# yl4579/StyleTTS2

Hardware: AMD Instinct MI355X
Metric: audio-seconds/sec (RTF^-1) end-to-end, 10 s utterance batch (higher is better)
Workload: dtype f32 (convs/linears: f16 hi/lo split, 3 MFMA products, fp32 accumulate)

## Files before the change

### include/st2.h

```cpp
#ifndef ST2_H
#define ST2_H

#include <stdint.h>

#ifdef __cplusplus
extern "C" {
#endif

#define ST2_ABI_VERSION 23

int st2_abi_version(void);
const char* st2_last_error(void);
int st2_device_info(int dev, char* name, int cap);

#define ST2_STATUS_F16_RANGE 1
#define ST2_STATUS_LSTM_TIMEOUT 2
#define ST2_STATUS_DURATION_SUM 4
#define ST2_STATUS_LSTM_RECOVERED 8
#define ST2_STATUS_FRAME_CAPACITY 16
int st2_status(int clear);

enum st2_prologue {
  ST2_PRO_NONE = 0,
  ST2_PRO_LEAKY = 1,
// ... 275 lines not shown
int st2_durations_fit(const int64_t* dur, int32_t B, int32_t N, const int32_t* len, const int32_t* target, const uint8_t* hold,
                      int32_t T_cap, int64_t* out, int32_t* report, void* stream);

int64_t st2_clip_ingest_work_bytes(int32_t B, int32_t L_cap);
int st2_clip_ingest(const void* src, int64_t src_bs, const int32_t* n, int32_t B, int32_t N_cap, int32_t fmt, int32_t up,
                    int32_t down, const float* taps, int32_t taps_per_phase, float top_db, int32_t L_min, float* wave,
                    int64_t w_bs, int32_t L_cap, int32_t* len, int32_t* start, int32_t* flags, void* work, int64_t work_bytes,
                    void* stream);

int st2_stft_frames(const float* wave, int64_t w_bs, int32_t B, int32_t L, int32_t n_win, int32_t hop, int32_t shift,
                    float* frames, int64_t f_bs, int32_t f_cs, void* stream);
int st2_power_spectrum(const float* y, int64_t y_bs, int32_t y_cs, int32_t B, int32_t K, int32_t M, float* p,
                       int64_t p_bs, int32_t p_cs, void* stream);
int st2_log_norm(float* x, int64_t n, float eps, float mean, float stdv, void* stream);
int st2_dwconv3x3s2(const float* x, int64_t x_bs, int64_t x_hs, int32_t x_cs, const float* w, const float* bias,
                    int32_t B, int32_t C, int32_t H, int32_t W, float* y, int64_t y_bs, int64_t y_hs, int32_t y_cs,
                    void* stream);
int st2_avgpool2x2(const float* x, int64_t x_bs, int64_t x_hs, int32_t x_cs, int32_t B, int32_t C, int32_t H, int32_t W,
                   float* y, int64_t y_bs, int64_t y_hs, int32_t y_cs, void* stream);

int st2_axpbypcz(const float* x, float a, const float* y, float b, const float* z, float c,
                 float* out, int64_t n, void* stream);

typedef struct st2_engine st2_engine;

typedef struct st2_model_config {
  int32_t decoder_kind;
  int32_t dim_in;
  int32_t style_dim;
  int32_t upsample_initial_channel;
  int32_t n_upsamples;  int32_t upsample_rates[4];  int32_t upsample_kernel_sizes[4];
  int32_t n_resblock_kernels;  int32_t resblock_kernel_sizes[4];  int32_t resblock_dilations[4][3];
  int32_t gen_istft_n_fft, gen_istft_hop;
  int32_t multispeaker;
  int32_t dn_layers, dn_heads, dn_head_features, dn_multiplier;
  int32_t dn_channels;
  int32_t dn_embedding;
  int32_t dn_context_features;
  int32_t dn_max_length;
  int32_t pred_hidden;
  int32_t bert_layers;
  float bert_ln_eps;
} st2_model_config;

int st2_create(const st2_model_config* cfg, st2_engine** out);
int st2_destroy(st2_engine* e);
// ... 184 lines not shown
```

### styletts2_amd/_lib.py

```python
import ctypes as C
import os

import torch

_HERE = os.path.dirname(os.path.abspath(__file__))
LIB_PATH = os.path.join(_HERE, "libst2_hip.so")
ABI_VERSION = 23
HEADROOM_COLS, CALIBRATION_COLS = 12, 5

f32p = C.c_void_p

PRO_NONE, PRO_LEAKY, PRO_ADAIN_LEAKY, PRO_ADAIN_SNAKE, PRO_SNAKE, PRO_COLNORM = range(6)
STATUS_F16_RANGE, STATUS_LSTM_TIMEOUT, STATUS_DURATION_SUM, STATUS_LSTM_RECOVERED = 1, 2, 4, 8
STATUS_FRAME_CAPACITY = 16
PACK_F32, PACK_S16 = 0, 1
PCM_F32, PCM_S16, PCM_ULAW, PCM_ALAW = range(4)
NOISE_NORMAL, NOISE_BITS = 0, 1
NOISE_SAMPLER, NOISE_STEP, NOISE_SINE = 0, 1, 0x10000
ACT_NONE, ACT_GELU, ACT_EXP_SIN, ACT_TANH, ACT_LEAKY, ACT_GELU_TANH = range(6)


class ConvDesc(C.Structure):
    _fields_ = [
        ("B", C.c_int32), ("C_in", C.c_int32), ("C_out", C.c_int32), ("L_in", C.c_int32),
# ... 294 lines not shown
    "st2_probe_mfma_stream": (C.c_int, [C.c_int32, C.c_int32, C.c_int32, C.c_void_p]),
    "st2_debug_headroom": (C.c_int, [C.c_int]),
    "st2_debug_headroom_read": (C.c_int, [C.POINTER(C.c_double), C.c_int32]),
    "st2_conv1d_xs_part_cols": (C.c_int, [C.POINTER(ConvDesc)]),
    "st2_conv1d_f16s_set_splitk": (None, [C.c_int, C.c_int]),
    "st2_calibrate": (C.c_int, [C.c_void_p, C.c_int32, C.POINTER(C.c_int32)]),
    "st2_calibration_read": (C.c_int, [C.c_void_p, C.POINTER(C.c_double), C.c_int32]),
    "st2_calibration_site_name": (C.c_int, [C.c_void_p, C.c_int32, C.c_char_p, C.c_int32]),
    "st2_calibration_write": (C.c_int, [C.c_void_p, C.POINTER(C.c_float), C.c_int32]),
    "st2_calibration_scale": (C.c_float, [C.c_float, C.c_int32]),
    "st2_stream_create_cu_mask": (C.c_int, [C.POINTER(C.c_uint32), C.c_int32, C.POINTER(C.c_void_p)]),
    "st2_stream_destroy": (C.c_int, [C.c_void_p]),
    "st2_debug_set_backend": (C.c_int, [C.POINTER(C.c_void_p), C.c_int32]),
    "st2_stft_frames": (C.c_int, [f32p, C.c_int64, C.c_int32, C.c_int32, C.c_int32, C.c_int32, C.c_int32, f32p,
                                  C.c_int64, C.c_int32, C.c_void_p]),
    "st2_power_spectrum": (C.c_int, [f32p, C.c_int64, C.c_int32, C.c_int32, C.c_int32, C.c_int32, f32p, C.c_int64,
                                     C.c_int32, C.c_void_p]),
    "st2_log_norm": (C.c_int, [f32p, C.c_int64, C.c_float, C.c_float, C.c_float, C.c_void_p]),
    "st2_dwconv3x3s2": (C.c_int, [f32p, C.c_int64, C.c_int64, C.c_int32, f32p, f32p, C.c_int32, C.c_int32, C.c_int32,
                                  C.c_int32, f32p, C.c_int64, C.c_int64, C.c_int32, C.c_void_p]),
    "st2_avgpool2x2": (C.c_int, [f32p, C.c_int64, C.c_int64, C.c_int32, C.c_int32, C.c_int32, C.c_int32, C.c_int32, f32p,
                                 C.c_int64, C.c_int64, C.c_int32, C.c_void_p]),
    "st2_axpbypcz": (C.c_int, [f32p, C.c_float, f32p, C.c_float, f32p, C.c_float, f32p, C.c_int64, C.c_void_p]),
    "st2_stft_frames_len": (C.c_int, [f32p, C.c_int64, C.c_int32, C.c_int32, C.c_int32, C.c_int32, C.c_int32, f32p,
                                      C.c_int64, C.c_int32, C.c_void_p, C.c_int32, C.c_void_p, C.c_void_p]),
    "st2_log_norm_len": (C.c_int, [f32p, C.c_int64, C.c_int32, C.c_int32, C.c_int32, C.c_int32, C.c_float, C.c_float,
                                   C.c_float, C.c_void_p, C.c_void_p]),
    "st2_dwconv3x3s2_len": (C.c_int, [f32p, C.c_int64, C.c_int64, C.c_int32, f32p, f32p, C.c_int32, C.c_int32, C.c_int32,
                                      C.c_int32, f32p, C.c_int64, C.c_int64, C.c_int32, C.c_void_p, C.c_void_p]),
    "st2_avgpool2x2_len": (C.c_int, [f32p, C.c_int64, C.c_int64, C.c_int32, C.c_int32, C.c_int32, C.c_int32, C.c_int32, f32p,
                                     C.c_int64, C.c_int64, C.c_int32, C.c_void_p, C.c_void_p]),
    "st2_style_lengths_count": (C.c_int64, [C.c_int32, C.c_int32, C.c_int32]),
    "st2_style_lengths": (C.c_int, [C.c_void_p, C.c_int32, C.c_int32, C.c_int32, C.c_int32, C.c_int32, C.c_void_p,
                                    C.c_void_p]),
    "st2_style_workspace_bytes_ragged": (C.c_int64, [C.c_void_p, C.c_int32, C.c_int32, C.c_int32, C.c_int32]),
    "st2_style_forward_ragged": (C.c_int, [C.c_void_p, C.c_int32, f32p, C.c_void_p, C.c_int32, C.c_int32, C.c_int32, f32p,
                                           C.c_void_p, C.c_int64, C.c_void_p]),
    "st2_conv_launch_plan": (C.c_int, [C.POINTER(ConvDesc), C.c_int32, C.c_int32, C.c_int32, C.POINTER(ConvPlan)]),
    "st2_convt_interleave_part_cols": (C.c_int, []),
}

EXPORTS = tuple(_SIGNATURES)
_lib = None


class St2Error(RuntimeError):
# ... 44 lines not shown
```

### styletts2_amd/csrc/st2_glue.hip

```cpp
#include <string.h>

#include "st2_common.h"

namespace {

__global__ __launch_bounds__(256) void time_features_kernel(float t, const float* __restrict__ w, int H2, int B,
                                                            float* __restrict__ out) {
  const int j = blockIdx.x * 256 + threadIdx.x;
  const int b = blockIdx.y;
  const int W = 1 + 2 * H2;
  if (j >= W) return;
  float v;
  if (j == 0) {
    v = t;
  } else {
    const int k = (j - 1) % H2;
    const float f = ((t * w[k]) * 2.0f) * 3.14159274101257324f;
    v = (j - 1) < H2 ? sinf(f) : cosf(f);
  }
  out[(int64_t)b * W + j] = v;
}

__global__ __launch_bounds__(256) void tokens_to_channels_kernel(const float* __restrict__ e, int64_t e_bs, int N, int E,
                                                                 float* __restrict__ y, int64_t y_bs, int y_cs) {
// ... 155 lines not shown
  const int tx = threadIdx.x & 31, ty = threadIdx.x >> 5;
  const int nlen = len ? len[b] : N;
#pragma unroll
  for (int i = 0; i < 4; ++i) {
    const int n = n0 + ty + 8 * i, e = e0 + tx;
    float v = 0.f;
    if (n < N && n < nlen && e < E) {
      const long long t = tok[(int64_t)b * N + n];
      if (t >= 0 && t < V) v = table[t * E + e];
      if (add) v += add[e];
      if (pos) v += pos[(int64_t)n * E + e];
    }
    tile[ty + 8 * i][tx] = v;
  }
  __syncthreads();
  float* yb = y + (int64_t)b * y_bs;
#pragma unroll
  for (int i = 0; i < 4; ++i) {
    const int e = e0 + ty + 8 * i, n = n0 + tx;
    if (n < N && e < E) yb[(int64_t)e * y_cs + n] = tile[tx][ty + 8 * i];
  }
}

}

extern "C" int st2_embed_tokens(const int64_t* tokens, int32_t B, int32_t N, const float* table, int32_t V, int32_t E,
                                const float* add, const float* pos, const int32_t* len, float* y, int64_t y_bs,
                                int32_t y_cs, void* stream) {
  ST2_REQUIRE(tokens && table && y && B > 0 && N > 0 && V > 0 && E > 0, "st2_embed_tokens: bad arguments");
  ST2_REQUIRE(B <= 65535, "st2_embed_tokens: grid too large");
  hipLaunchKernelGGL(embed_tokens_kernel, dim3(st2_cdiv(N, 32), st2_cdiv(E, 32), B), dim3(256), 0,
                     reinterpret_cast<hipStream_t>(stream), reinterpret_cast<const long long*>(tokens), table, V, E, N, add,
                     pos, len, y, y_bs, y_cs);
  ST2_CHECK_LAUNCH("st2_embed_tokens");
  return 0;
}

extern "C" int st2_mask_tail(float* x, int64_t x_bs, int32_t x_cs, int32_t B, int32_t C, int32_t L, const int32_t* len,
                             void* stream) {
  ST2_REQUIRE(x && len && B > 0 && C > 0 && L > 0, "st2_mask_tail: bad arguments");
  ST2_REQUIRE(B <= 65535 && C <= 65535, "st2_mask_tail: grid too large");
  hipLaunchKernelGGL(mask_tail_kernel, dim3(st2_cdiv(L, 256), C, B), dim3(256), 0, reinterpret_cast<hipStream_t>(stream), x,
                     x_bs, x_cs, L, len);
  ST2_CHECK_LAUNCH("st2_mask_tail");
  return 0;
}
// ... 113 lines not shown
```

### styletts2_amd/csrc/st2_norm.hip

```cpp
#include "st2_common.h"

namespace {

template <int NT>
__global__ __launch_bounds__(NT) void instnorm_stats_kernel(const float* __restrict__ x, int64_t x_bs, int x_cs,
                                                            int C, int L_max, float eps, float* __restrict__ stats,
                                                            const int32_t* __restrict__ len) {
  const int row = blockIdx.x;
  const int b = row / C;
  const int c = row % C;
  const int L = len ? min(max(len[b], 1), L_max) : L_max;
  const float* xr = x + (int64_t)b * x_bs + (int64_t)c * x_cs;
  double s = 0.0, ss = 0.0;
  if ((reinterpret_cast<uintptr_t>(xr) & 15) == 0) {
    typedef float f4 __attribute__((ext_vector_type(4)));
    double a[4] = {0.0, 0.0, 0.0, 0.0}, q[4] = {0.0, 0.0, 0.0, 0.0};
    const int L4 = L >> 2;
    const f4* x4 = reinterpret_cast<const f4*>(xr);
    for (int i = threadIdx.x; i < L4; i += NT) {
      const f4 v = x4[i];
#pragma unroll
      for (int e = 0; e < 4; ++e) {
        const double d = (double)v[e];
        a[e] += d;
// ... 37 lines not shown
  __shared__ double red[2][NT / 64];
  const int lane = threadIdx.x & 63, wave = threadIdx.x >> 6;
  if (lane == 0) {
    red[0][wave] = s;
    red[1][wave] = ss;
  }
  __syncthreads();
  if (threadIdx.x == 0) {
    double ts = 0.0, tss = 0.0;
#pragma unroll
    for (int w = 0; w < NT / 64; ++w) {
      ts += red[0][w];
      tss += red[1][w];
    }
    const double mean = ts / (double)L;
    double var = tss / (double)L - mean * mean;
    if (var < 0.0) var = 0.0;
    stats[(int64_t)row * 2 + 0] = (float)mean;
    stats[(int64_t)row * 2 + 1] = (float)(1.0 / sqrt(var + (double)eps));
  }
}

constexpr int CW = 16;
__global__ __launch_bounds__(64 * CW) void colnorm_stats_kernel(const float* __restrict__ x, int64_t x_bs, int x_cs,
                                                                int C, int L, float eps, float* __restrict__ stats) {
  __shared__ double red[2][CW][64];
  const int lane = threadIdx.x & 63;
  const int w = threadIdx.x >> 6;
  const int l = blockIdx.x * 64 + lane;
  const int b = blockIdx.y;
  const bool live = l < L;
  const float* xb = x + (int64_t)b * x_bs + (live ? l : 0);
  double s = 0.0, ss = 0.0;
  int c = w;
  for (; c + 7 * CW < C; c += 8 * CW) {
    float v[8];
#pragma unroll
    for (int u = 0; u < 8; ++u) v[u] = xb[(int64_t)(c + u * CW) * x_cs];
#pragma unroll
    for (int u = 0; u < 8; ++u) {
      const double dv = (double)v[u];
      s += dv;
      ss += dv * dv;
    }
  }
  for (; c < C; c += CW) {
    const double dv = (double)xb[(int64_t)c * x_cs];
    s += dv;
    ss += dv * dv;
  }
  red[0][w][lane] = s;
  red[1][w][lane] = ss;
  __syncthreads();
  if (w == 0 && live) {
    double ts = 0.0, tss = 0.0;
#pragma unroll
    for (int i = 0; i < CW; ++i) {
      ts += red[0][i][lane];
      tss += red[1][i][lane];
    }
    const double mean = ts / (double)C;
    double var = tss / (double)C - mean * mean;
    if (var < 0.0) var = 0.0;
    float* o = stats + ((int64_t)b * L + l) * 2;
    o[0] = (float)mean;
    o[1] = (float)(1.0 / sqrt(var + (double)eps));
  }
}

constexpr int FC_BT = 8;
constexpr int FC_J = 64;
constexpr int FC_KS = 16;
constexpr int FC_NT = FC_J * FC_KS;
__global__ __launch_bounds__(FC_NT) void style_fc_kernel(const float* __restrict__ s, int B, int K,
                                                       const float* __restrict__ wt, const float* __restrict__ bias,
                                                       int J, int act, float* __restrict__ h) {
  extern __shared__ __attribute__((aligned(16))) float sl[];
  float* red = sl + FC_BT * K;
  const int jj = threadIdx.x & (FC_J - 1);
  const int ks = threadIdx.x / FC_J;
  const int j = blockIdx.x * FC_J + jj;
  const int jc = min(j, J - 1);
  const int b0 = blockIdx.y * FC_BT;
  const int nb = min(FC_BT, B - b0);
  for (int e = threadIdx.x; e < FC_BT * K; e += FC_NT) {
    const int bb = e / K, k = e % K;
    sl[e] = bb < nb ? s[(int64_t)(b0 + bb) * K + k] : 0.f;
  }
  __syncthreads();
  float acc[FC_BT];
// ... 96 lines not shown
extern "C" int st2_instnorm_stats_len(const float* x, int64_t x_bs, int32_t x_cs, int32_t B, int32_t C, int32_t L,
                                      float eps, float* stats, const int32_t* len, void* stream) {
  ST2_REQUIRE(x && stats && B > 0 && C > 0 && L > 0, "st2_instnorm_stats: bad arguments");
  hipStream_t s = reinterpret_cast<hipStream_t>(stream);
  const int rows = B * C;
  if (L <= 2048)
    hipLaunchKernelGGL((instnorm_stats_kernel<64>), dim3(rows), dim3(64), 0, s, x, x_bs, x_cs, C, L, eps, stats, len);
  else
    hipLaunchKernelGGL((instnorm_stats_kernel<256>), dim3(rows), dim3(256), 0, s, x, x_bs, x_cs, C, L, eps, stats, len);
  ST2_CHECK_LAUNCH("st2_instnorm_stats");
  return 0;
}

extern "C" int st2_colnorm_stats(const float* x, int64_t x_bs, int32_t x_cs, int32_t B, int32_t C, int32_t L,
                                 float eps, float* stats, void* stream) {
  ST2_REQUIRE(x && stats && B > 0 && C > 0 && L > 0, "st2_colnorm_stats: bad arguments");
  hipStream_t s = reinterpret_cast<hipStream_t>(stream);
  hipLaunchKernelGGL(colnorm_stats_kernel, dim3(st2_cdiv(L, 64), B), dim3(64 * CW), 0, s, x, x_bs, x_cs, C, L, eps,
                     stats);
  ST2_CHECK_LAUNCH("st2_colnorm_stats");
  return 0;
}

extern "C" int st2_style_fc(const float* sv, int32_t B, int32_t K, const float* wt, const float* bias, int32_t J,
                            int32_t act, float* h, void* stream) {
  ST2_REQUIRE(sv && wt && h && B > 0 && K > 0 && J > 0, "st2_style_fc: bad arguments");
  ST2_REQUIRE(K <= 2048, "st2_style_fc: K=%d too large", K);
  ST2_REQUIRE(act == ST2_ACT_NONE || act == ST2_ACT_GELU, "st2_style_fc: act must be NONE or GELU");
  hipStream_t s = reinterpret_cast<hipStream_t>(stream);
  const size_t smem = ((size_t)FC_BT * K + (size_t)FC_KS * FC_BT * FC_J) * sizeof(float);
  static std::atomic<uint64_t> attr_done{0};
  st2_once_per_device(attr_done, [&] {
    (void)hipFuncSetAttribute(reinterpret_cast<const void*>(&style_fc_kernel), hipFuncAttributeMaxDynamicSharedMemorySize,
                              160 * 1024);
  });
  hipLaunchKernelGGL(style_fc_kernel, dim3(st2_cdiv(J, FC_J), st2_cdiv(B, FC_BT)), dim3(FC_NT), smem, s, sv, B, K, wt,
                     bias, J, act, h);
  ST2_CHECK_LAUNCH("st2_style_fc");
  return 0;
}
```

### styletts2_amd/csrc/st2_plan_sampler.inc

```

struct Sess {
  Ctx& c;
  const st2_engine& e;
  int B, N;
  bool merged;
  const int32_t* key_len;
  View bases[2];
  int nbases;
  const float* feat_map;
  const float* ada;
  double scale;
};

View dn_alloc(Sess& s, int C) {
  View v;
  v.B = s.B; v.C = C; v.L = s.N;
  v.p = s.c.a.f32((int64_t)s.B * C * s.N);
  if (s.merged) { v.bs = s.N; v.cs = s.B * s.N; } else { v.bs = (int64_t)C * s.N; v.cs = s.N; }
  return v;
}
View dn_cv(const Sess& s, const View& t) {
  if (!s.merged) return t;
  View v = t;
  v.B = 1; v.L = s.B * s.N; v.bs = (int64_t)t.C * v.L; v.cs = v.L;
  return v;
}

const float* dn_mapping(Sess& s, float c_noise) {
  Ctx& c = s.c;
  const st2_engine& e = s.e;
  const PDenoiser& d = e.dn;
  const int F = d.features, H2 = e.cfg.dn_channels / 2;
  float* four = c.a.f32((int64_t)s.B * (1 + 2 * H2));
  RUN(c, g_be.time_features(c_noise, e.F(d.time_w), H2, s.B, four, c.stream));
  float* m = c.a.f32((int64_t)s.B * F);
  RUN(c, g_be.style_fc(four, s.B, 1 + 2 * H2, e.F(d.time_lin), e.F(d.time_b), F, ST2_ACT_GELU, m, c.stream));
  if (s.feat_map) {
    float* m2 = c.a.f32((int64_t)s.B * F);
    RUN(c, g_be.axpbypcz(m, 1.0f, s.feat_map, 1.0f, nullptr, 0.0f, m2, (int64_t)s.B * F, c.stream));
    m = m2;
  }
  float* m3 = c.a.f32((int64_t)s.B * F);
  RUN(c, g_be.style_fc(m, s.B, F, e.F(d.map0), e.F(d.map0_b), F, ST2_ACT_GELU, m3, c.stream));
  float* m4 = c.a.f32((int64_t)s.B * F);
  RUN(c, g_be.style_fc(m3, s.B, F, e.F(d.map2), e.F(d.map2_b), F, ST2_ACT_GELU, m4, c.stream));
  return m4;
}

void dn_run(Sess& s, View base, const float* x, const float* m, float* out) {
  Ctx& c = s.c;
  const st2_engine& e = s.e;
  const PDenoiser& d = e.dn;
  const st2_model_config& cfg = e.cfg;
  const int B = s.B, N = s.N, Fz = d.features, C = cfg.dn_channels;
  const int mid = cfg.dn_heads * cfg.dn_head_features;
  const int64_t mark = c.a.off;
  View b0 = base.rows(0, C);
  RUN(c, g_be.broadcast_cols(x, C, b0.p, b0.bs, b0.cs, B, C, N, c.stream));
  View X = dn_alloc(s, Fz);
  RUN(c, g_be.add_chanvec(base.p, base.bs, base.cs, m, Fz, X.p, X.bs, X.cs, B, Fz, N, c.stream));
  const int nblk = (int)d.blocks.size();
  for (int i = 0; i < nblk; ++i) {
    const PBlock& b = d.blocks[(size_t)i];
    float* st = c.a.f32((int64_t)B * N * 2);
    RUN(c, g_be.colnorm_stats(X.p, X.bs, X.cs, B, Fz, N, 1e-5f, st, c.stream));
    View qkv = dn_alloc(s, 3 * mid);
    ConvOpt o1, o2;
    o1.pro = o2.pro = ST2_PRO_COLNORM;
    o1.stats = o2.stats = st;
    if (cfg.multispeaker) {
      const int64_t J = (int64_t)nblk * 4 * Fz;
      const float* a = s.ada + (int64_t)4 * Fz * i;
      o1.gamma = a;          o1.beta = a + Fz;     o1.gb_bs = J; o1.gamma_plus_one = 1;
      o2.gamma = a + 2 * Fz; o2.beta = a + 3 * Fz; o2.gb_bs = J; o2.gamma_plus_one = 1;
    } else {
      o1.gamma = e.F(b.n_w);  o1.beta = e.F(b.n_b);
      o2.gamma = e.F(b.nc_w); o2.beta = e.F(b.nc_b);
    }
    const bool seg = cfg.multispeaker && s.merged && B > 1 &&
                     conv_rule(ST2_PRO_COLNORM, 1, 1, Fz, mid, B * N).route == ST2_CONV_ROUTE_XS;
    if (seg) o1.gb_seg = o2.gb_seg = N;
    const bool per_utt = cfg.multispeaker && !seg;
    View Xv = per_utt ? X : dn_cv(s, X), qv = per_utt ? qkv : dn_cv(s, qkv);
    conv(c, e, Xv, b.q, qv.rows(0, mid), o1);
    conv(c, e, Xv, b.kv, qv.rows(mid, 3 * mid), o2);
    View att = dn_alloc(s, mid);
    View q = qkv.rows(0, mid), k = qkv.rows(mid, 2 * mid), v = qkv.rows(2 * mid, 3 * mid);
    RUN(c, g_be.attention_keylen(q.p, k.p, v.p, q.bs, q.cs, att.p, att.bs, att.cs, B, cfg.dn_heads, cfg.dn_head_features,
                                 N, (float)pow((double)cfg.dn_head_features, -0.5), s.key_len, c.stream));
    View X1 = dn_alloc(s, Fz), hmid = dn_alloc(s, b.f1_out), X2 = dn_alloc(s, Fz);
    ConvOpt oo;
    oo.bias = e.F(b.o_b); oo.res = dn_cv(s, X);
    conv(c, e, dn_cv(s, att), b.o, dn_cv(s, X1), oo);
    ConvOpt of1;
    of1.bias = e.F(b.f1_b); of1.act = ST2_ACT_GELU;
    conv(c, e, dn_cv(s, X1), b.f1, dn_cv(s, hmid), of1);
    ConvOpt of2;
    of2.bias = e.F(b.f2_b); of2.res = dn_cv(s, X1);
    conv(c, e, dn_cv(s, hmid), b.f2, dn_cv(s, X2), of2);
    if (i + 1 < nblk) {
      View Xn = dn_alloc(s, Fz);
      RUN(c, g_be.add_chanvec(X2.p, X2.bs, X2.cs, m, Fz, Xn.p, Xn.bs, Xn.cs, B, Fz, N, c.stream));
      X = Xn;
    } else {
      X = X2;
    }
  }
  float* mean = c.a.f32((int64_t)B * Fz);
  RUN(c, g_be.mean_tokens_len(X.p, X.bs, X.cs, mean, Fz, B, Fz, N, s.key_len, c.stream));
  RUN(c, g_be.style_fc(mean, B, Fz, e.F(d.out_t), e.F(d.out_b), C, ST2_ACT_NONE, out, c.stream));
  c.a.off = mark;
}

void dn_denoise(Sess& s, const float* x, const double* w4, float* out) {
  Ctx& c = s.c;
  const int C = s.e.cfg.dn_channels;
  const int64_t n = (int64_t)s.B * C;
  const int64_t mark = c.a.off;
  const float c_skip = (float)w4[0], c_out = (float)w4[1], c_in = (float)w4[2], c_noise = (float)w4[3];
  float* x_in = c.a.f32(n);
  RUN(c, g_be.axpbypcz(x, c_in, nullptr, 0.f, nullptr, 0.f, x_in, n, c.stream));
  const float* m = dn_mapping(s, c_noise);
  float* pred = c.a.f32(n);
  dn_run(s, s.bases[0], x_in, m, pred);
  if (s.nbases > 1) {
    float* pm = c.a.f32(n);
    dn_run(s, s.bases[1], x_in, m, pm);
    float* mix = c.a.f32(n);
    RUN(c, g_be.axpbypcz(pm, (float)(1.0 - s.scale), pred, (float)s.scale, nullptr, 0.f, mix, n, c.stream));
    pred = mix;
  }
  RUN(c, g_be.axpbypcz(x, c_skip, pred, c_out, nullptr, 0.f, out, n, c.stream));
  c.a.off = mark;
}

int sampler_plan(Ctx& c, const st2_engine& e, const float* noise, const float* embedding, const View* emb_cm,
                 const float* features, const float* step_noise, const int32_t* lengths, int B, int N, int steps, double scale,
                 const double* table, double sigma0, float* out, float* step_taps) {
  const st2_model_config& cfg = e.cfg;
  const PDenoiser& d = e.dn;
  const int C = cfg.dn_channels, E = cfg.dn_embedding, Fz = d.features;
  Sess s{c, e, B, N, true, lengths, {}, 1, nullptr, nullptr, scale};
  s.bases[0] = dn_alloc(s, Fz);
  {
    View dst = s.bases[0].rows(C, Fz);
    if (emb_cm)
      RUN(c, g_be.copy_ncl(emb_cm->p, emb_cm->bs, emb_cm->cs, dst.p, dst.bs, dst.cs, B, E, N, c.stream));
    else
      RUN(c, g_be.tokens_to_channels(embedding, (int64_t)N * E, B, N, E, dst.p, dst.bs, dst.cs, c.stream));
  }
  if (scale != 1.0) {
    s.nbases = 2;
    s.bases[1] = dn_alloc(s, Fz);
    View dst = s.bases[1].rows(C, Fz);
    RUN(c, g_be.tokens_to_channels(e.F(d.fixed), 0, B, N, E, dst.p, dst.bs, dst.cs, c.stream));
  }
  if (cfg.multispeaker) {
    if (!features) { st2_set_error("st2_sampler_run: the multispeaker denoiser needs `features`"); return 1; }
    float* fm = c.a.f32((int64_t)B * Fz);
    RUN(c, g_be.style_fc(features, B, cfg.dn_context_features, e.F(d.feat), e.F(d.feat_b), Fz, ST2_ACT_GELU, fm, c.stream));
    const int J = cfg.dn_layers * 4 * Fz;
    float* ada = c.a.f32((int64_t)B * J);
    RUN(c, g_be.style_fc(features, B, cfg.dn_context_features, e.F(d.ada_wt), e.F(d.ada_b), J, ST2_ACT_NONE, ada, c.stream));
    s.feat_map = fm;
    s.ada = ada;
  }
  const int64_t n = (int64_t)B * C;
  float* xa = c.a.f32(n);
  float* xb = c.a.f32(n);
  float* x = xa;
  RUN(c, g_be.axpbypcz(noise, (float)sigma0, nullptr, 0.f, nullptr, 0.f, x, n, c.stream));
  for (int i = 0; i + 1 < steps; ++i) {
    const double* row = table + (int64_t)i * ST2_SAMPLER_TABLE_COLS;
    const int64_t mark = c.a.off;
    float* den = c.a.f32(n);
    dn_denoise(s, x, row + 0, den);
    const double k = row[8];
    float* x_mid = c.a.f32(n);
    RUN(c, g_be.axpbypcz(x, (float)(1.0 + k), den, (float)(-k), nullptr, 0.f, x_mid, n, c.stream));
    float* den_mid = c.a.f32(n);
    dn_denoise(s, x_mid, row + 4, den_mid);
    const double k2 = row[9];
    float* d_mid = c.a.f32(n);
    RUN(c, g_be.axpbypcz(x_mid, (float)k2, den_mid, (float)(-k2), nullptr, 0.f, d_mid, n, c.stream));
    float* xn = (x == xa) ? xb : xa;
    RUN(c, g_be.axpbypcz(x, 1.0f, d_mid, 1.0f, step_noise + (int64_t)i * n, (float)row[10], xn, n, c.stream));
    x = xn;
    if (step_taps) RUN(c, g_be.axpbypcz(x, 1.0f, nullptr, 0.f, nullptr, 0.f, step_taps + (int64_t)i * n, n, c.stream));
    c.a.off = mark;
  }
  RUN(c, g_be.axpbypcz(x, 1.0f, nullptr, 0.f, nullptr, 0.f, out, n, c.stream));
  return c.rc;
}
```

### styletts2_amd/ops.py

```python
import ctypes as C
import json
import warnings

import torch

from . import _hooks, _lib
from .weights import F16S_X_SCALE, SplitConvWeight
from ._lib import (ACT_EXP_SIN, ACT_GELU, ACT_GELU_TANH, ACT_LEAKY, ACT_NONE, ACT_TANH, PRO_ADAIN_LEAKY, PRO_ADAIN_SNAKE,
                   PRO_COLNORM, PRO_LEAKY, PRO_NONE, PRO_SNAKE, ConvDesc)


def _stream():
    return C.c_void_p(torch.cuda.current_stream().cuda_stream)


_AUX_STREAMS = {}


def aux_stream(dev, priority=0, index=0):
    dev = torch.device(dev)
    key = (dev.index if dev.index is not None else torch.cuda.current_device(), int(priority), int(index))
    if key not in _AUX_STREAMS:
        _AUX_STREAMS[key] = torch.cuda.Stream(dev, priority=int(priority))
    return _AUX_STREAMS[key]
# ... 741 lines not shown
    lp = _chk_len(lengths, "lengths", B, x)
    if out is None:
        out = torch.empty((B, Cc), device=x.device, dtype=torch.float32)
    _lib.check(lib.st2_mean_tokens_len(x.data_ptr(), x.stride(0), x.stride(1), out.data_ptr(), out.stride(0), B, Cc, N, lp,
                                       _stream()), "st2_mean_tokens")
    return out


def axpbypcz(x, a, y=None, b=0.0, z=None, c=0.0, out=None):
    lib = _lib.load()
    _chk(x, "x")
    assert x.is_contiguous()
    for t in (y, z):
        if t is not None:
            _chk(t, "operand")
            assert t.is_contiguous() and t.numel() == x.numel()
    if out is None:
        out = torch.empty_like(x)
    _lib.check(lib.st2_axpbypcz(x.data_ptr(), a, _ptr(y), b, _ptr(z), c, out.data_ptr(), x.numel(), _stream()),
               "st2_axpbypcz")
    return out


def time_features(t, w, B, out=None):
    lib = _lib.load()
    _chk(w, "w", 1)
    H2 = w.numel()
    if out is None:
        out = torch.empty((B, 1 + 2 * H2), device=w.device, dtype=torch.float32)
    _lib.check(lib.st2_time_features(float(t), w.data_ptr(), H2, B, out.data_ptr(), _stream()), "st2_time_features")
    return out


def tokens_to_channels(e, out, B=None):
    lib = _lib.load()
    _chk(e, "e")
    _chk(out, "out", 3)
    assert e.is_contiguous()
    if e.dim() == 2:
        N, E = e.shape
        e_bs = 0
        B = out.shape[0] if B is None else B
    else:
        B, N, E = e.shape
        e_bs = N * E
    assert out.shape[0] == B and out.shape[1] == E and out.shape[2] == N, (out.shape, (B, E, N))
# ... 694 lines not shown
```

Before: 5044.

## Fuse diffusion sampler elementwise steps, batch time mappings, and compose colnorm stats

Adds fused ADPM2 mid/end kernels that combine the guidance blend, denoise, step update, noise addition and next-input scaling into one pass each. The time-embedding MLP for all sampler calls is now computed once as a batched style_fc up front. The broadcast, add_chanvec and colnorm_stats sequence in each denoiser block is merged into one kernel that writes the composed tensor while reducing its statistics. The aim is fewer kernel launches and less memory traffic in the sampler loop. The fused path is taken only when the default HIP backend is active, and the new composed kernel uses a narrower 16-column tile than the original colnorm kernel.

New measurement: 5056, median of 6. No clear change (+0.2%).

```diff
diff --git a/include/st2.h b/include/st2.h
--- a/include/st2.h
+++ b/include/st2.h
@@ -321,6 +321,15 @@
 int st2_axpbypcz(const float* x, float a, const float* y, float b, const float* z, float c,
                  float* out, int64_t n, void* stream);
 
+int st2_compose_colnorm_stats(const float* x, int64_t x_bs, int32_t x_cs, const float* head, int32_t C0, const float* v,
+                              int64_t v_bs, float* y, int64_t y_bs, int32_t y_cs, int32_t B, int32_t C, int32_t L, float eps,
+                              float* stats, void* stream);
+int st2_adpm2_mid(const float* x, const float* pred, const float* pm, float w_pm, float w_pred, float c_skip, float c_out,
+                  float a_x, float a_den, float c_in, float* x_mid, float* x_in, int64_t n, void* stream);
+int st2_adpm2_end(const float* x, const float* x_mid, const float* pred, const float* pm, float w_pm, float w_pred,
+                  float c_skip, float c_out, float a_mid, float a_den, const float* eps, float s_up, float c_in,
+                  float* x_next, float* x_in, float* tap, float* out, int64_t n, void* stream);
+
 typedef struct st2_engine st2_engine;
 
 typedef struct st2_model_config {
diff --git a/styletts2_amd/_lib.py b/styletts2_amd/_lib.py
--- a/styletts2_amd/_lib.py
+++ b/styletts2_amd/_lib.py
@@ -340,6 +340,11 @@
     "st2_avgpool2x2": (C.c_int, [f32p, C.c_int64, C.c_int64, C.c_int32, C.c_int32, C.c_int32, C.c_int32, C.c_int32, f32p,
                                  C.c_int64, C.c_int64, C.c_int32, C.c_void_p]),
     "st2_axpbypcz": (C.c_int, [f32p, C.c_float, f32p, C.c_float, f32p, C.c_float, f32p, C.c_int64, C.c_void_p]),
+    "st2_compose_colnorm_stats": (C.c_int, [f32p, C.c_int64, C.c_int32, f32p, C.c_int32, f32p, C.c_int64, f32p, C.c_int64,
+                                            C.c_int32, C.c_int32, C.c_int32, C.c_int32, C.c_float, f32p, C.c_void_p]),
+    "st2_adpm2_mid": (C.c_int, [f32p, f32p, f32p] + [C.c_float] * 7 + [f32p, f32p, C.c_int64, C.c_void_p]),
+    "st2_adpm2_end": (C.c_int, [f32p, f32p, f32p, f32p] + [C.c_float] * 6 + [f32p, C.c_float, C.c_float, f32p, f32p, f32p, f32p,
+                                C.c_int64, C.c_void_p]),
     "st2_stft_frames_len": (C.c_int, [f32p, C.c_int64, C.c_int32, C.c_int32, C.c_int32, C.c_int32, C.c_int32, f32p,
                                       C.c_int64, C.c_int32, C.c_void_p, C.c_int32, C.c_void_p, C.c_void_p]),
     "st2_log_norm_len": (C.c_int, [f32p, C.c_int64, C.c_int32, C.c_int32, C.c_int32, C.c_int32, C.c_float, C.c_float,
diff --git a/styletts2_amd/csrc/st2_glue.hip b/styletts2_amd/csrc/st2_glue.hip
--- a/styletts2_amd/csrc/st2_glue.hip
+++ b/styletts2_amd/csrc/st2_glue.hip
@@ -201,6 +201,73 @@
   }
 }
 
+__device__ __forceinline__ float adpm2_pred(const float* __restrict__ pred, const float* __restrict__ pm, float w_pm, float w_pred,
+                                            int64_t i) {
+  if (!pm) return pred[i];
+  float p = w_pm * pm[i];
+  p += w_pred * pred[i];
+  return p;
+}
+
+__global__ __launch_bounds__(256) void adpm2_mid_kernel(const float* __restrict__ x, const float* __restrict__ pred,
+                                                        const float* __restrict__ pm, float w_pm, float w_pred, float c_skip,
+                                                        float c_out, float a_x, float a_den, float c_in, float* __restrict__ x_mid,
+                                                        float* __restrict__ x_in, int64_t n) {
+  const int64_t i = (int64_t)blockIdx.x * 256 + threadIdx.x;
+  if (i >= n) return;
+  const float p = adpm2_pred(pred, pm, w_pm, w_pred, i);
+  float den = c_skip * x[i];
+  den += c_out * p;
+  float xm = a_x * x[i];
+  xm += a_den * den;
+  x_mid[i] = xm;
+  x_in[i] = c_in * xm;
+}
+
+__global__ __launch_bounds__(256) void adpm2_end_kernel(const float* __restrict__ x, const float* __restrict__ x_mid,
+                                                        const float* __restrict__ pred, const float* __restrict__ pm, float w_pm,
+                                                        float w_pred, float c_skip, float c_out, float a_mid, float a_den,
+                                                        const float* __restrict__ eps, float s_up, float c_in,
+                                                        float* __restrict__ x_next, float* __restrict__ x_in,
+                                                        float* __restrict__ tap, float* __restrict__ out, int64_t n) {
+  const int64_t i = (int64_t)blockIdx.x * 256 + threadIdx.x;
+  if (i >= n) return;
+  const float p = adpm2_pred(pred, pm, w_pm, w_pred, i);
+  float den = c_skip * x_mid[i];
+  den += c_out * p;
+  float d = a_mid * x_mid[i];
+  d += a_den * den;
+  float v = 1.0f * x[i];
+  v += 1.0f * d;
+  v += s_up * eps[i];
+  x_next[i] = v;
+  if (tap) tap[i] = 1.0f * v;
+  if (out) out[i] = 1.0f * v;
+  if (x_in) x_in[i] = c_in * v;
+}
+
+}
+
+extern "C" int st2_adpm2_mid(const float* x, const float* pred, const float* pm, float w_pm, float w_pred, float c_skip, float c_out,
+                             float a_x, float a_den, float c_in, float* x_mid, float* x_in, int64_t n, void* stream) {
+  ST2_REQUIRE(x && pred && x_mid && x_in && n > 0, "st2_adpm2_mid: x / pred / x_mid / x_in is NULL, or n=%lld", (long long)n);
+  ST2_REQUIRE(x_mid != x && x_in != x && x_in != x_mid, "st2_adpm2_mid: the outputs must be buffers of their own");
+  hipLaunchKernelGGL(adpm2_mid_kernel, dim3(st2_cdiv(n, 256)), dim3(256), 0, reinterpret_cast<hipStream_t>(stream), x, pred, pm, w_pm,
+                     w_pred, c_skip, c_out, a_x, a_den, c_in, x_mid, x_in, n);
+  ST2_CHECK_LAUNCH("st2_adpm2_mid");
+  return 0;
+}
+
+extern "C" int st2_adpm2_end(const float* x, const float* x_mid, const float* pred, const float* pm, float w_pm, float w_pred,
+                             float c_skip, float c_out, float a_mid, float a_den, const float* eps, float s_up, float c_in,
+                             float* x_next, float* x_in, float* tap, float* out, int64_t n, void* stream) {
+  ST2_REQUIRE(x && x_mid && pred && eps && x_next && n > 0, "st2_adpm2_end: x / x_mid / pred / eps / x_next is NULL, or n=%lld",
+              (long long)n);
+  ST2_REQUIRE(x_next != x && x_next != x_mid && x_in != x && x_in != x_mid, "st2_adpm2_end: the outputs must be buffers of their own");
+  hipLaunchKernelGGL(adpm2_end_kernel, dim3(st2_cdiv(n, 256)), dim3(256), 0, reinterpret_cast<hipStream_t>(stream), x, x_mid, pred, pm,
+                     w_pm, w_pred, c_skip, c_out, a_mid, a_den, eps, s_up, c_in, x_next, x_in, tap, out, n);
+  ST2_CHECK_LAUNCH("st2_adpm2_end");
+  return 0;
 }
 
 extern "C" int st2_embed_tokens(const int64_t* tokens, int32_t B, int32_t N, const float* table, int32_t V, int32_t E,
diff --git a/styletts2_amd/csrc/st2_norm.hip b/styletts2_amd/csrc/st2_norm.hip
--- a/styletts2_amd/csrc/st2_norm.hip
+++ b/styletts2_amd/csrc/st2_norm.hip
@@ -83,21 +83,17 @@
 }
 
 constexpr int CW = 16;
-__global__ __launch_bounds__(64 * CW) void colnorm_stats_kernel(const float* __restrict__ x, int64_t x_bs, int x_cs,
-                                                                int C, int L, float eps, float* __restrict__ stats) {
-  __shared__ double red[2][CW][64];
-  const int lane = threadIdx.x & 63;
-  const int w = threadIdx.x >> 6;
-  const int l = blockIdx.x * 64 + lane;
-  const int b = blockIdx.y;
-  const bool live = l < L;
-  const float* xb = x + (int64_t)b * x_bs + (live ? l : 0);
+template <int TL, class Load>
+__device__ __forceinline__ void colnorm_reduce(Load load, int C, float eps, bool live, float* __restrict__ o) {
+  __shared__ double red[2][CW][TL];
+  const int lane = threadIdx.x % TL;
+  const int w = threadIdx.x / TL;
   double s = 0.0, ss = 0.0;
   int c = w;
   for (; c + 7 * CW < C; c += 8 * CW) {
     float v[8];
 #pragma unroll
-    for (int u = 0; u < 8; ++u) v[u] = xb[(int64_t)(c + u * CW) * x_cs];
+    for (int u = 0; u < 8; ++u) v[u] = load(c + u * CW);
 #pragma unroll
     for (int u = 0; u < 8; ++u) {
       const double dv = (double)v[u];
@@ -106,7 +102,7 @@
     }
   }
   for (; c < C; c += CW) {
-    const double dv = (double)xb[(int64_t)c * x_cs];
+    const double dv = (double)load(c);
     s += dv;
     ss += dv * dv;
   }
@@ -123,10 +119,41 @@
     const double mean = ts / (double)C;
     double var = tss / (double)C - mean * mean;
     if (var < 0.0) var = 0.0;
-    float* o = stats + ((int64_t)b * L + l) * 2;
     o[0] = (float)mean;
     o[1] = (float)(1.0 / sqrt(var + (double)eps));
   }
+}
+
+__global__ __launch_bounds__(64 * CW) void colnorm_stats_kernel(const float* __restrict__ x, int64_t x_bs, int x_cs,
+                                                                int C, int L, float eps, float* __restrict__ stats) {
+  const int l = blockIdx.x * 64 + (threadIdx.x & 63);
+  const int b = blockIdx.y;
+  const bool live = l < L;
+  const float* xb = x + (int64_t)b * x_bs + (live ? l : 0);
+  colnorm_reduce<64>([&](int c) { return xb[(int64_t)c * x_cs]; }, C, eps, live, stats + ((int64_t)b * L + (live ? l : 0)) * 2);
+}
+
+constexpr int CT = 16;
+__global__ __launch_bounds__(CT * CW) void compose_colnorm_stats_kernel(const float* __restrict__ x, int64_t x_bs, int x_cs,
+                                                                        const float* __restrict__ head, int C0,
+                                                                        const float* __restrict__ v, int64_t v_bs,
+                                                                        float* __restrict__ y, int64_t y_bs, int y_cs, int C,
+                                                                        int L, float eps, float* __restrict__ stats) {
+  const int l = blockIdx.x * CT + (threadIdx.x % CT);
+  const int b = blockIdx.y;
+  const bool live = l < L;
+  const int lc = live ? l : 0;
+  const float* xb = x + (int64_t)b * x_bs + lc;
+  const float* hb = head + (int64_t)b * C0;
+  const float* vb = v + (int64_t)b * v_bs;
+  float* yb = y + (int64_t)b * y_bs + lc;
+  colnorm_reduce<CT>(
+      [&](int c) {
+        const float t = (c < C0 ? hb[c] : xb[(int64_t)c * x_cs]) + vb[c];
+        if (live) yb[(int64_t)c * y_cs] = t;
+        return t;
+      },
+      C, eps, live, stats + ((int64_t)b * L + lc) * 2);
 }
 
 constexpr int FC_BT = 8;
@@ -269,6 +296,20 @@
   return 0;
 }
 
+extern "C" int st2_compose_colnorm_stats(const float* x, int64_t x_bs, int32_t x_cs, const float* head, int32_t C0, const float* v,
+                                         int64_t v_bs, float* y, int64_t y_bs, int32_t y_cs, int32_t B, int32_t C, int32_t L,
+                                         float eps, float* stats, void* stream) {
+  ST2_REQUIRE(x && v && y && stats && x != y, "st2_compose_colnorm_stats: x / v / y / stats is NULL (or y is x)");
+  ST2_REQUIRE(B > 0 && C > 0 && L > 0 && C0 >= 0 && C0 <= C && (C0 == 0 || head),
+              "st2_compose_colnorm_stats: bad geometry (B=%d, C=%d, L=%d, C0=%d%s)", B, C, L, C0, C0 > 0 && !head ? ", head is NULL" : "");
+  ST2_REQUIRE(B <= 65535, "st2_compose_colnorm_stats: grid too large");
+  hipStream_t s = reinterpret_cast<hipStream_t>(stream);
+  hipLaunchKernelGGL(compose_colnorm_stats_kernel, dim3(st2_cdiv(L, CT), B), dim3(CT * CW), 0, s, x, x_bs, x_cs, head, C0, v, v_bs, y,
+                     y_bs, y_cs, C, L, eps, stats);
+  ST2_CHECK_LAUNCH("st2_compose_colnorm_stats");
+  return 0;
+}
+
 extern "C" int st2_style_fc(const float* sv, int32_t B, int32_t K, const float* wt, const float* bias, int32_t J,
                             int32_t act, float* h, void* stream) {
   ST2_REQUIRE(sv && wt && h && B > 0 && K > 0 && J > 0, "st2_style_fc: bad arguments");
diff --git a/styletts2_amd/csrc/st2_plan_sampler.inc b/styletts2_amd/csrc/st2_plan_sampler.inc
--- a/styletts2_amd/csrc/st2_plan_sampler.inc
+++ b/styletts2_amd/csrc/st2_plan_sampler.inc
@@ -10,6 +10,7 @@
   const float* feat_map;
   const float* ada;
   double scale;
+  bool fused = false;
 };
 
 View dn_alloc(Sess& s, int C) {
@@ -26,25 +27,52 @@
   return v;
 }
 
-const float* dn_mapping(Sess& s, float c_noise) {
+const float* dn_mappings(Sess& s, const double* table, int calls) {
   Ctx& c = s.c;
   const st2_engine& e = s.e;
   const PDenoiser& d = e.dn;
-  const int F = d.features, H2 = e.cfg.dn_channels / 2;
-  float* four = c.a.f32((int64_t)s.B * (1 + 2 * H2));
-  RUN(c, g_be.time_features(c_noise, e.F(d.time_w), H2, s.B, four, c.stream));
-  float* m = c.a.f32((int64_t)s.B * F);
-  RUN(c, g_be.style_fc(four, s.B, 1 + 2 * H2, e.F(d.time_lin), e.F(d.time_b), F, ST2_ACT_GELU, m, c.stream));
+  const int F = d.features, H2 = e.cfg.dn_channels / 2, W = 1 + 2 * H2;
+  const int R = calls * s.B;
+  float* m4 = c.a.f32((int64_t)R * F);
+  const int64_t mark = c.a.off;
+  float* four = c.a.f32((int64_t)R * W);
+  for (int j = 0; j < calls; ++j) {
+    const float c_noise = (float)table[(int64_t)(j / 2) * ST2_SAMPLER_TABLE_COLS + (j % 2) * 4 + 3];
+    RUN(c, g_be.time_features(c_noise, e.F(d.time_w), H2, s.B, four + (int64_t)j * s.B * W, c.stream));
+  }
+  float* m = c.a.f32((int64_t)R * F);
+  RUN(c, g_be.style_fc(four, R, W, e.F(d.time_lin), e.F(d.time_b), F, ST2_ACT_GELU, m, c.stream));
   if (s.feat_map) {
-    float* m2 = c.a.f32((int64_t)s.B * F);
-    RUN(c, g_be.axpbypcz(m, 1.0f, s.feat_map, 1.0f, nullptr, 0.0f, m2, (int64_t)s.B * F, c.stream));
+    float* m2 = c.a.f32((int64_t)R * F);
+    for (int j = 0; j < calls; ++j) {
+      const int64_t o = (int64_t)j * s.B * F;
+      RUN(c, g_be.axpbypcz(m + o, 1.0f, s.feat_map, 1.0f, nullptr, 0.0f, m2 + o, (int64_t)s.B * F, c.stream));
+    }
     m = m2;
   }
-  float* m3 = c.a.f32((int64_t)s.B * F);
-  RUN(c, g_be.style_fc(m, s.B, F, e.F(d.map0), e.F(d.map0_b), F, ST2_ACT_GELU, m3, c.stream));
-  float* m4 = c.a.f32((int64_t)s.B * F);
-  RUN(c, g_be.style_fc(m3, s.B, F, e.F(d.map2), e.F(d.map2_b), F, ST2_ACT_GELU, m4, c.stream));
+  float* m3 = c.a.f32((int64_t)R * F);
+  RUN(c, g_be.style_fc(m, R, F, e.F(d.map0), e.F(d.map0_b), F, ST2_ACT_GELU, m3, c.stream));
+  RUN(c, g_be.style_fc(m3, R, F, e.F(d.map2), e.F(d.map2_b), F, ST2_ACT_GELU, m4, c.stream));
+  c.a.off = mark;
   return m4;
+}
+
+bool sampler_fused() {
+  return g_be.broadcast_cols == kHipBackend.broadcast_cols && g_be.add_chanvec == kHipBackend.add_chanvec &&
+         g_be.colnorm_stats == kHipBackend.colnorm_stats && g_be.axpbypcz == kHipBackend.axpbypcz &&
+         g_be.time_features == kHipBackend.time_features && g_be.style_fc == kHipBackend.style_fc;
+}
+
+void dn_compose_stats(Sess& s, const View& src, const float* head, int C0, const float* m, const View& X, float* st) {
+  Ctx& c = s.c;
+  const int B = s.B, N = s.N, Fz = X.C;
+  if (s.fused) {
+    RUN(c, st2_compose_colnorm_stats(src.p, src.bs, src.cs, head, C0, m, Fz, X.p, X.bs, X.cs, B, Fz, N, 1e-5f, st, c.stream));
+    return;
+  }
+  if (C0 > 0) RUN(c, g_be.broadcast_cols(head, C0, src.p, src.bs, src.cs, B, C0, N, c.stream));
+  RUN(c, g_be.add_chanvec(src.p, src.bs, src.cs, m, Fz, X.p, X.bs, X.cs, B, Fz, N, c.stream));
+  RUN(c, g_be.colnorm_stats(X.p, X.bs, X.cs, B, Fz, N, 1e-5f, st, c.stream));
 }
 
 void dn_run(Sess& s, View base, const float* x, const float* m, float* out) {
@@ -55,15 +83,13 @@
   const int B = s.B, N = s.N, Fz = d.features, C = cfg.dn_channels;
   const int mid = cfg.dn_heads * cfg.dn_head_features;
   const int64_t mark = c.a.off;
-  View b0 = base.rows(0, C);
-  RUN(c, g_be.broadcast_cols(x, C, b0.p, b0.bs, b0.cs, B, C, N, c.stream));
   View X = dn_alloc(s, Fz);
-  RUN(c, g_be.add_chanvec(base.p, base.bs, base.cs, m, Fz, X.p, X.bs, X.cs, B, Fz, N, c.stream));
+  View src = base;
   const int nblk = (int)d.blocks.size();
   for (int i = 0; i < nblk; ++i) {
     const PBlock& b = d.blocks[(size_t)i];
     float* st = c.a.f32((int64_t)B * N * 2);
-    RUN(c, g_be.colnorm_stats(X.p, X.bs, X.cs, B, Fz, N, 1e-5f, st, c.stream));
+    dn_compose_stats(s, src, i == 0 ? x : nullptr, i == 0 ? C : 0, m, X, st);
     View qkv = dn_alloc(s, 3 * mid);
     ConvOpt o1, o2;
     o1.pro = o2.pro = ST2_PRO_COLNORM;
@@ -98,18 +124,34 @@
     ConvOpt of2;
     of2.bias = e.F(b.f2_b); of2.res = dn_cv(s, X1);
     conv(c, e, dn_cv(s, hmid), b.f2, dn_cv(s, X2), of2);
-    if (i + 1 < nblk) {
-      View Xn = dn_alloc(s, Fz);
-      RUN(c, g_be.add_chanvec(X2.p, X2.bs, X2.cs, m, Fz, Xn.p, Xn.bs, Xn.cs, B, Fz, N, c.stream));
-      X = Xn;
-    } else {
-      X = X2;
-    }
+    src = X2;
+    X = i + 1 < nblk ? dn_alloc(s, Fz) : X2;
   }
   float* mean = c.a.f32((int64_t)B * Fz);
   RUN(c, g_be.mean_tokens_len(X.p, X.bs, X.cs, mean, Fz, B, Fz, N, s.key_len, c.stream));
   RUN(c, g_be.style_fc(mean, B, Fz, e.F(d.out_t), e.F(d.out_b), C, ST2_ACT_NONE, out, c.stream));
   c.a.off = mark;
+}
+
+const float* dn_mapping(Sess& s, float c_noise) {
+  Ctx& c = s.c;
+  const st2_engine& e = s.e;
+  const PDenoiser& d = e.dn;
+  const int F = d.features, H2 = e.cfg.dn_channels / 2;
+  float* four = c.a.f32((int64_t)s.B * (1 + 2 * H2));
+  RUN(c, g_be.time_features(c_noise, e.F(d.time_w), H2, s.B, four, c.stream));
+  float* m = c.a.f32((int64_t)s.B * F);
+  RUN(c, g_be.style_fc(four, s.B, 1 + 2 * H2, e.F(d.time_lin), e.F(d.time_b), F, ST2_ACT_GELU, m, c.stream));
+  if (s.feat_map) {
+    float* m2 = c.a.f32((int64_t)s.B * F);
+    RUN(c, g_be.axpbypcz(m, 1.0f, s.feat_map, 1.0f, nullptr, 0.0f, m2, (int64_t)s.B * F, c.stream));
+    m = m2;
+  }
+  float* m3 = c.a.f32((int64_t)s.B * F);
+  RUN(c, g_be.style_fc(m, s.B, F, e.F(d.map0), e.F(d.map0_b), F, ST2_ACT_GELU, m3, c.stream));
+  float* m4 = c.a.f32((int64_t)s.B * F);
+  RUN(c, g_be.style_fc(m3, s.B, F, e.F(d.map2), e.F(d.map2_b), F, ST2_ACT_GELU, m4, c.stream));
+  return m4;
 }
 
 void dn_denoise(Sess& s, const float* x, const double* w4, float* out) {
@@ -134,38 +176,10 @@
   c.a.off = mark;
 }
 
-int sampler_plan(Ctx& c, const st2_engine& e, const float* noise, const float* embedding, const View* emb_cm,
-                 const float* features, const float* step_noise, const int32_t* lengths, int B, int N, int steps, double scale,
-                 const double* table, double sigma0, float* out, float* step_taps) {
-  const st2_model_config& cfg = e.cfg;
-  const PDenoiser& d = e.dn;
-  const int C = cfg.dn_channels, E = cfg.dn_embedding, Fz = d.features;
-  Sess s{c, e, B, N, true, lengths, {}, 1, nullptr, nullptr, scale};
-  s.bases[0] = dn_alloc(s, Fz);
-  {
-    View dst = s.bases[0].rows(C, Fz);
-    if (emb_cm)
-      RUN(c, g_be.copy_ncl(emb_cm->p, emb_cm->bs, emb_cm->cs, dst.p, dst.bs, dst.cs, B, E, N, c.stream));
-    else
-      RUN(c, g_be.tokens_to_channels(embedding, (int64_t)N * E, B, N, E, dst.p, dst.bs, dst.cs, c.stream));
-  }
-  if (scale != 1.0) {
-    s.nbases = 2;
-    s.bases[1] = dn_alloc(s, Fz);
-    View dst = s.bases[1].rows(C, Fz);
-    RUN(c, g_be.tokens_to_channels(e.F(d.fixed), 0, B, N, E, dst.p, dst.bs, dst.cs, c.stream));
-  }
-  if (cfg.multispeaker) {
-    if (!features) { st2_set_error("st2_sampler_run: the multispeaker denoiser needs `features`"); return 1; }
-    float* fm = c.a.f32((int64_t)B * Fz);
-    RUN(c, g_be.style_fc(features, B, cfg.dn_context_features, e.F(d.feat), e.F(d.feat_b), Fz, ST2_ACT_GELU, fm, c.stream));
-    const int J = cfg.dn_layers * 4 * Fz;
-    float* ada = c.a.f32((int64_t)B * J);
-    RUN(c, g_be.style_fc(features, B, cfg.dn_context_features, e.F(d.ada_wt), e.F(d.ada_b), J, ST2_ACT_NONE, ada, c.stream));
-    s.feat_map = fm;
-    s.ada = ada;
-  }
-  const int64_t n = (int64_t)B * C;
+void sampler_steps_per_kernel(Sess& s, const float* noise, const float* step_noise, int steps, const double* table, double sigma0,
+                              float* out, float* step_taps) {
+  Ctx& c = s.c;
+  const int64_t n = (int64_t)s.B * s.e.cfg.dn_channels;
   float* xa = c.a.f32(n);
   float* xb = c.a.f32(n);
   float* x = xa;
@@ -190,5 +204,92 @@
     c.a.off = mark;
   }
   RUN(c, g_be.axpbypcz(x, 1.0f, nullptr, 0.f, nullptr, 0.f, out, n, c.stream));
+}
+
+struct Pred {
+  float* pred;
+  float* pm;
+};
+Pred dn_net(Sess& s, const float* x_in, const float* m) {
+  Ctx& c = s.c;
+  const int64_t n = (int64_t)s.B * s.e.cfg.dn_channels;
+  Pred p{c.a.f32(n), nullptr};
+  dn_run(s, s.bases[0], x_in, m, p.pred);
+  if (s.nbases > 1) {
+    p.pm = c.a.f32(n);
+    dn_run(s, s.bases[1], x_in, m, p.pm);
+  }
+  return p;
+}
+
+void sampler_steps_fused(Sess& s, const float* noise, const float* step_noise, int steps, const double* table, double sigma0,
+                         float* out, float* step_taps) {
+  Ctx& c = s.c;
+  const int Fz = s.e.dn.features;
+  const float* maps = dn_mappings(s, table, 2 * (steps - 1));
+  const int64_t n = (int64_t)s.B * s.e.cfg.dn_channels, mrows = (int64_t)s.B * Fz;
+  const float w_pm = (float)(1.0 - s.scale), w_pred = (float)s.scale;
+  float* xa = c.a.f32(n);
+  float* xb = c.a.f32(n);
+  float* x_in = c.a.f32(n);
+  float* x_in_mid = c.a.f32(n);
+  float* x_mid = c.a.f32(n);
+  float* x = xa;
+  RUN(c, g_be.axpbypcz(noise, (float)sigma0, nullptr, 0.f, nullptr, 0.f, x, n, c.stream));
+  RUN(c, g_be.axpbypcz(x, (float)table[2], nullptr, 0.f, nullptr, 0.f, x_in, n, c.stream));
+  for (int i = 0; i + 1 < steps; ++i) {
+    const double* row = table + (int64_t)i * ST2_SAMPLER_TABLE_COLS;
+    const bool last = i + 2 == steps;
+    const int64_t mark = c.a.off;
+    const Pred p = dn_net(s, x_in, maps + (int64_t)(2 * i) * mrows);
+    RUN(c, st2_adpm2_mid(x, p.pred, p.pm, w_pm, w_pred, (float)row[0], (float)row[1], (float)(1.0 + row[8]), (float)(-row[8]),
+                         (float)row[6], x_mid, x_in_mid, n, c.stream));
+    c.a.off = mark;
+    const Pred q = dn_net(s, x_in_mid, maps + (int64_t)(2 * i + 1) * mrows);
+    float* xn = (x == xa) ? xb : xa;
+    RUN(c, st2_adpm2_end(x, x_mid, q.pred, q.pm, w_pm, w_pred, (float)row[4], (float)row[5], (float)row[9], (float)(-row[9]),
+                         step_noise + (int64_t)i * n, (float)row[10], last ? 0.f : (float)row[ST2_SAMPLER_TABLE_COLS + 2], xn,
+                         last ? nullptr : x_in, step_taps ? step_taps + (int64_t)i * n : nullptr, last ? out : nullptr, n, c.stream));
+    x = xn;
+    c.a.off = mark;
+  }
+}
+
+int sampler_plan(Ctx& c, const st2_engine& e, const float* noise, const float* embedding, const View* emb_cm,
+                 const float* features, const float* step_noise, const int32_t* lengths, int B, int N, int steps, double scale,
+                 const double* table, double sigma0, float* out, float* step_taps) {
+  const st2_model_config& cfg = e.cfg;
+  const PDenoiser& d = e.dn;
+  const int C = cfg.dn_channels, E = cfg.dn_embedding, Fz = d.features;
+  Sess s{c, e, B, N, true, lengths, {}, 1, nullptr, nullptr, scale};
+  s.fused = sampler_fused();
+  s.bases[0] = dn_alloc(s, Fz);
+  {
+    View dst = s.bases[0].rows(C, Fz);
+    if (emb_cm)
+      RUN(c, g_be.copy_ncl(emb_cm->p, emb_cm->bs, emb_cm->cs, dst.p, dst.bs, dst.cs, B, E, N, c.stream));
+    else
+      RUN(c, g_be.tokens_to_channels(embedding, (int64_t)N * E, B, N, E, dst.p, dst.bs, dst.cs, c.stream));
+  }
+  if (scale != 1.0) {
+    s.nbases = 2;
+    s.bases[1] = dn_alloc(s, Fz);
+    View dst = s.bases[1].rows(C, Fz);
+    RUN(c, g_be.tokens_to_channels(e.F(d.fixed), 0, B, N, E, dst.p, dst.bs, dst.cs, c.stream));
+  }
+  if (cfg.multispeaker) {
+    if (!features) { st2_set_error("st2_sampler_run: the multispeaker denoiser needs `features`"); return 1; }
+    float* fm = c.a.f32((int64_t)B * Fz);
+    RUN(c, g_be.style_fc(features, B, cfg.dn_context_features, e.F(d.feat), e.F(d.feat_b), Fz, ST2_ACT_GELU, fm, c.stream));
+    const int J = cfg.dn_layers * 4 * Fz;
+    float* ada = c.a.f32((int64_t)B * J);
+    RUN(c, g_be.style_fc(features, B, cfg.dn_context_features, e.F(d.ada_wt), e.F(d.ada_b), J, ST2_ACT_NONE, ada, c.stream));
+    s.feat_map = fm;
+    s.ada = ada;
+  }
+  if (s.fused)
+    sampler_steps_fused(s, noise, step_noise, steps, table, sigma0, out, step_taps);
+  else
+    sampler_steps_per_kernel(s, noise, step_noise, steps, table, sigma0, out, step_taps);
   return c.rc;
 }
diff --git a/styletts2_amd/ops.py b/styletts2_amd/ops.py
--- a/styletts2_amd/ops.py
+++ b/styletts2_amd/ops.py
@@ -787,6 +787,56 @@
     return out
 
 
+def compose_colnorm_stats(x, v, head=None, out=None, stats=None, eps=1e-5):
+    lib = _lib.load()
+    _chk(x, "x", 3)
+    _chk(v, "v", 2)
+    B, Cc, L = x.shape
+    assert v.shape == (B, Cc) and v.stride(1) == 1
+    C0 = 0
+    if head is not None:
+        _chk(head, "head", 2)
+        assert head.is_contiguous() and head.shape[0] == B and head.shape[1] <= Cc
+        C0 = head.shape[1]
+    if out is None:
+        out = torch.empty((B, Cc, L), device=x.device, dtype=torch.float32)
+    if stats is None:
+        stats = torch.empty((B, L, 2), device=x.device, dtype=torch.float32)
+    assert out.shape == x.shape and stats.is_contiguous() and stats.numel() == B * L * 2
+    _lib.check(lib.st2_compose_colnorm_stats(x.data_ptr(), x.stride(0), x.stride(1), _ptr(head), C0, v.data_ptr(), v.stride(0),
+                                             out.data_ptr(), out.stride(0), out.stride(1), B, Cc, L, eps, stats.data_ptr(),
+                                             _stream()), "st2_compose_colnorm_stats")
+    return out, stats
+
+
+def _flat(t, name, n):
+    _chk(t, name)
+    assert t.is_contiguous() and t.numel() == n
+    return t.data_ptr()
+
+
+def adpm2_mid(x, pred, pm, w_pm, w_pred, c_skip, c_out, a_x, a_den, c_in):
+    lib = _lib.load()
+    n = x.numel()
+    x_mid, x_in = torch.empty_like(x), torch.empty_like(x)
+    _lib.check(lib.st2_adpm2_mid(_flat(x, "x", n), _flat(pred, "pred", n), 0 if pm is None else _flat(pm, "pm", n), w_pm, w_pred,
+                                 c_skip, c_out, a_x, a_den, c_in, x_mid.data_ptr(), x_in.data_ptr(), n, _stream()), "st2_adpm2_mid")
+    return x_mid, x_in
+
+
+def adpm2_end(x, x_mid, pred, pm, w_pm, w_pred, c_skip, c_out, a_mid, a_den, eps, s_up, c_in, want_in=True, want_tap=False,
+              want_out=False):
+    lib = _lib.load()
+    n = x.numel()
+    x_next = torch.empty_like(x)
+    x_in, tap, out = (torch.empty_like(x) if w else None for w in (want_in, want_tap, want_out))
+    _lib.check(lib.st2_adpm2_end(_flat(x, "x", n), _flat(x_mid, "x_mid", n), _flat(pred, "pred", n),
+                                 0 if pm is None else _flat(pm, "pm", n), w_pm, w_pred, c_skip, c_out, a_mid, a_den,
+                                 _flat(eps, "eps", n), s_up, c_in, x_next.data_ptr(), _ptr(x_in), _ptr(tap), _ptr(out), n, _stream()),
+               "st2_adpm2_end")
+    return x_next, x_in, tap, out
+
+
 def time_features(t, w, B, out=None):
     lib = _lib.load()
     _chk(w, "w", 1)
```
